# angela000/DQNFlappyBird

Hardware: AMD Instinct MI355X
Metric: env steps/sec (whole node) + DQN grad-steps/sec, 80x80x4 batch=32 (higher is better)
Workload: dtype f32

## Files before the change

### dqnflappybird_amd/csrc/fb_qnet.hip

```cpp
#include <math.h>
#include <stdlib.h>
#include "fb_common.h"

#ifndef FK_ABL
#define FK_ABL 0
#endif
#ifndef BW_ABL
#define BW_ABL 0
#endif

namespace {

typedef float f32x16 __attribute__((ext_vector_type(16)));

constexpr int OFF_W1 = 0, OFF_B1 = 8192, OFF_W2 = 8224, OFF_B2 = 40992, OFF_W3 = 41056, OFF_B3 = 77920,
              OFF_WF1 = 77984;
constexpr int CONV_PARAMS = OFF_WF1;
#include "fb_head.h"
#include "fb_sampler.h"
#include "fb_gather.h"
constexpr int MAXTB = 256;


struct Slice { const float *params; const uint8_t *states; int s_off, count; const uint16_t *w1s; int fshift; };
// ... 1607 lines not shown

__global__ __launch_bounds__(256) void noisy_sigma_init_kernel(float *__restrict__ p, NoisyNet N) {
    const int q = OFF_WF1 + blockIdx.x * 256 + threadIdx.x;
    if (q >= N.n) return;
    p[N.n + q - OFF_WF1] = noisy_layer(N, q).sig;
}

__device__ __forceinline__ float env_noise_f(uint32_t seed_lo, uint32_t seed_hi, uint32_t c0, uint32_t step_lo, uint32_t step_hi) {
    const fb_u4 r = fb_philox(seed_lo, seed_hi, c0, step_lo, FB_STREAM_ENV_NOISE, step_hi);
    const float u1 = ((r.x >> 8) + 1) * (1.0f / 16777216.0f), u2 = (r.y >> 8) * (1.0f / 16777216.0f);
    const float z = sqrtf(-2.f * logf(u1)) * cosf(6.28318530717958647692f * u2);
    return copysignf(sqrtf(fabsf(z)), z);
}

__global__ __launch_bounds__(256) void env_noise_sigsplit_kernel(const float *__restrict__ sig, uint4 *__restrict__ wsp, int FC, const AdamDev *ad,
                                                                const int *seen) {
    if (*seen == ad->applies) return;
    const int id = blockIdx.x * 256 + threadIdx.x;
    if (id < 200 * FC) wsplit_item(sig, wsp, FC, IT_CONV + id);
}

struct EnvScale { const uint16_t *a3; const float *h3; size_t pl; uint16_t *out; int n, nz; uint32_t seed_lo, seed_hi, step_lo, step_hi;
                  const AdamDev *ad; int *seen; unsigned *ovf; };
__global__ __launch_bounds__(256) void env_noise_scale_kernel(EnvScale a) {
    if (blockIdx.x == 0 && threadIdx.x == 0) *a.seen = a.ad->applies;
    const int id = blockIdx.x * 256 + threadIdx.x, e = min(id / 800, a.n - 1), k = 2 * (id - (id / 800) * 800);
    const bool on = id < a.n * 800;
    const size_t o = (size_t)e * 1600 + k;
    float x0, x1;
    if (a.a3) {
        const uint32_t hi = *reinterpret_cast<const uint32_t *>(a.a3 + o), lo = *reinterpret_cast<const uint32_t *>(a.a3 + a.pl + o);
        const f32x2 h = __builtin_convertvector(__builtin_bit_cast(f16x2, hi), f32x2), l = __builtin_convertvector(__builtin_bit_cast(f16x2, lo), f32x2);
        x0 = fmaf(l.x, F16_LO_UNSCALE, h.x); x1 = fmaf(l.y, F16_LO_UNSCALE, h.y);
    } else { x0 = a.h3[o]; x1 = a.h3[o + 1]; }
    const uint32_t c = (uint32_t)e * (uint32_t)a.nz + (uint32_t)k;
    const float y0 = x0 * env_noise_f(a.seed_lo, a.seed_hi, c, a.step_lo, a.step_hi), y1 = x1 * env_noise_f(a.seed_lo, a.seed_hi, c + 1u, a.step_lo, a.step_hi);
    uint32_t hi, lo;
    split2x2(y0, y1, hi, lo);
    if (on) { *reinterpret_cast<uint32_t *>(a.out + o) = hi; *reinterpret_cast<uint32_t *>(a.out + a.pl + o) = lo; }
    note_overflow(on && out_of_f16_range(y0, y1, 0.f, 0.f), a.ovf);
}

struct EnvNoiseHead {
    const float *hf, *ht; int stot, nks;
    const float *P; NetOff hoff; const float *sig; NetOff off; NoisyNet N;
    int n, FC, A; C51Sup sup; float *q; uint8_t *actions; float epsilon; uint32_t seed_lo, seed_hi, step_lo, step_hi;
    const int32_t *key_of; uint32_t stream;
};
constexpr int ENH_WAVES = 8;
template <int AT> struct EnhLds { static constexpr int KC = AT == 2 ? 64 : 16, PER = (KC * AT * 64 + 511) / 512, PERV = (KC * 64 + 511) / 512; };
template <int AT, bool DUEL>
__global__ __launch_bounds__(64 * ENH_WAVES) void env_noise_head_kernel(EnvNoiseHead H) {
    constexpr int KC = EnhLds<AT>::KC, PER = EnhLds<AT>::PER, PERV = EnhLds<AT>::PERV, WQ = KC * AT * 64;
    __shared__ float lw[2 * WQ + (DUEL ? KC * 64 : 0)];
    const int tid = threadIdx.x, lane = tid & 63, row = blockIdx.x * ENH_WAVES + (tid >> 6);
    const bool live = row < H.n;
    const int smp = live ? row : H.n - 1;
    const int A = AT == MAXA ? H.A : AT, N = H.sup.N, AN = A * N, il = lane < N ? lane : N - 1, FC = H.FC;
    const bool on = lane < N;
    const int key = H.key_of ? H.key_of[smp] : smp;
    const uint32_t base = (uint32_t)key * (uint32_t)H.N.nz;
    auto draw = [&](int k) { return env_noise_f(H.seed_lo, H.seed_hi, base + (uint32_t)k, H.step_lo, H.step_hi); };
    const NoisyLayer L0 = H.N.l[0], LV = H.N.l[1], LQ = H.N.l[DUEL ? 2 : 1];
    float lg[AT], ns[AT], nv = 0.f;
#pragma unroll
    for (int a = 0; a < AT; a++) { lg[a] = 0.f; ns[a] = 0.f; }
    float x = 0.f, xq = 0.f, xv = 0.f;
    for (int k0 = 0; k0 < FC; k0 += KC) {
        const int cq = KC * AN, cv = KC * N;
        const float *__restrict__ gm = H.P + H.hoff.wq + (size_t)k0 * AN, *__restrict__ gq = H.sig + H.off.wq + (size_t)k0 * AN;
        const float *__restrict__ gv = H.sig + H.off.wv + (size_t)k0 * N;
        float tm[PER], tq[PER], tv[DUEL ? PERV : 1];
#pragma unroll
        for (int r = 0; r < PER; r++) { const int i = min(tid + r * 512, cq - 1); tm[r] = gm[i]; tq[r] = gq[i]; }
        if (DUEL) {
#pragma unroll
            for (int r = 0; r < PERV; r++) tv[r] = gv[min(tid + r * 512, cv - 1)];
        }
        if (k0 % 64 == 0) {
            const int j = k0 + lane;
            float v = H.hf[(size_t)smp * FC + j], t[FC1_KS];
#pragma unroll
            for (int ks = 1; ks < FC1_KS; ks++) {
                const float y = H.hf[((size_t)(ks < H.nks ? ks : 0) * H.stot + smp) * FC + j];
                t[ks] = ks < H.nks ? y : 0.f;
            }
#pragma unroll
            for (int ks = 1; ks < FC1_KS; ks++) v += t[ks];
            const float pre = v + H.P[H.hoff.bf1 + j];
            float tt = H.ht[(size_t)smp * FC + j];
#pragma unroll
            for (int ks = 1; ks < FC1_SP_KS; ks++) tt += H.ht[((size_t)ks * H.stot + smp) * FC + j];
            x = fmaxf(pre + draw(L0.eout + j) * (tt + H.sig[H.off.bf1 + j]), 0.f);
            xq = x * draw(LQ.ein + j);
            xv = DUEL ? x * draw(LV.ein + j) : 0.f;
        }
        __syncthreads();
#pragma unroll
        for (int r = 0; r < PER; r++) { const int i = tid + r * 512; if (i < cq) { lw[i] = tm[r]; lw[WQ + i] = tq[r]; } }
        if (DUEL) {
#pragma unroll
            for (int r = 0; r < PERV; r++) { const int i = tid + r * 512; if (i < cv) lw[2 * WQ + i] = tv[r]; }
        }
        __syncthreads();
        const int kl = k0 % 64;
#pragma unroll 8
        for (int k = 0; k < KC; k++) {
            const float xs = rdlane(x, kl + k), xqs = rdlane(xq, kl + k);
#pragma unroll
            for (int a = 0; a < AT; a++) {
                const int o = k * AN + (a < A ? a : 0) * N + il;
                lg[a] = fmaf(xs, lw[o], lg[a]);
                ns[a] = fmaf(xqs, lw[WQ + o], ns[a]);
            }
            if (DUEL) nv = fmaf(rdlane(xv, kl + k), lw[2 * WQ + k * N + il], nv);
        }
    }
#pragma unroll
    for (int a = 0; a < AT; a++) lg[a] += H.P[H.hoff.bq + (a < A ? a : 0) * N + il];
    float nq[AT], mean = 0.f;
#pragma unroll
    for (int a = 0; a < AT; a++) {
        const int o = (a < A ? a : 0) * N + il;
        nq[a] = draw(LQ.eout + o) * (ns[a] + H.sig[H.off.bq + o]);
        if (a < A) mean += nq[a];
    }
    if (DUEL) {
        mean /= (float)A;
        const float vn = draw(LV.eout + il) * (nv + H.sig[H.off.bv + il]);
#pragma unroll
        for (int a = 0; a < AT; a++) lg[a] += (vn + nq[a]) - mean;
    } else {
#pragma unroll
        for (int a = 0; a < AT; a++) lg[a] += nq[a];
    }
    float qv[AT];
    const float z = H.sup.vmin + (float)(on ? lane : 0) * H.sup.dz;
    c51_q<AT>(lg, on, z, qv);
    if (lane == 0 && live) {
#pragma unroll
        for (int a = 0; a < AT; a++) if (a < A) H.q[(size_t)smp * A + a] = qv[a];
        int best = 0;
#pragma unroll
        for (int a = 1; a < AT; a++) if (a < A && qv[a] > qv[best]) best = a;
        const fb_u4 o = fb_philox(H.seed_lo, H.seed_hi, (uint32_t)key, H.step_lo, H.stream, H.step_hi);
        const float u = (float)(o.x >> 8) * (1.0f / 16777216.0f);
        if (u <= H.epsilon) best = (int)(((unsigned long long)o.y * (unsigned)A) >> 32);
        H.actions[smp] = (uint8_t)best;
    }
}

typedef float f32x4 __attribute__((ext_vector_type(4)));
struct FkArgs { Slices sl; const float *h3; float *hf; float *qpart; int FC, A, dueling, stot; NetOff off; };
constexpr int FK_ROW = 204;

__global__ __launch_bounds__(512) void fc1_fk_kernel(FkArgs a) {
    __shared__ float ast[8 * 16 * FK_ROW];
    __shared__ float red[8 * 4 * 64];
    const Slice s = a.sl.s[blockIdx.z];
    const int M = s.count, m0 = blockIdx.x * 16, n0 = blockIdx.y * 16;
    if (m0 >= M) return;
    const int lane = threadIdx.x & 63, wave = threadIdx.x >> 6, r = lane & 15, g = lane >> 4;
    const int kw = wave * 200;
    const float *bcol = s.params + OFF_WF1 + (size_t)(kw + 50 * g) * a.FC + n0 + r;
    float bv[50];
#pragma unroll
    for (int t = 0; t < 50; t++) bv[t] = bcol[(size_t)(FK_ABL == 2 ? 0 : t) * a.FC];
    float hb = s.params[a.off.bf1 + n0 + r], hw[MAXA + 1];
#pragma unroll
    for (int c = 0; c < MAXA; c++) hw[c] = s.params[a.off.wq + (n0 + r) * a.A + (c < a.A ? c : 0)];
    hw[MAXA] = s.params[(a.dueling ? a.off.wv : a.off.bf1) + n0 + r];
    float *mine = ast + wave * 16 * FK_ROW;
    float4 st[13];
#pragma unroll
    for (int i = 0; i < 13; i++) {
        const int idx = lane + 64 * i, row = idx < 800 ? idx / 50 : 0, c4 = idx < 800 ? idx - row * 50 : 0;
        const int mr = m0 + row < M ? m0 + row : M - 1;
        st[i] = *reinterpret_cast<const float4 *>(a.h3 + (size_t)(s.s_off + mr) * 1600 + kw + 4 * (FK_ABL == 3 ? 0 : c4));
    }
#pragma unroll
    for (int i = 0; i < 13; i++) {
        const int idx = lane + 64 * i, row = idx / 50, c4 = idx - row * 50;
        if (idx < 800) *reinterpret_cast<float4 *>(mine + row * FK_ROW + 4 * c4) = st[i];
    }
    __builtin_amdgcn_wave_barrier();
    asm volatile("s_waitcnt lgkmcnt(0)" ::: "memory");
    const float *arow = mine + r * FK_ROW + 50 * g;
    f32x4 acc0 = {0.f, 0.f, 0.f, 0.f}, acc1 = {0.f, 0.f, 0.f, 0.f};
    float2 av[25];
#pragma unroll
    for (int t = 0; t < 25; t++) av[t] = *reinterpret_cast<const float2 *>(arow + 2 * t);
#pragma unroll
    for (int t = 0; t < 25; t++) { keep(av[t].x); keep(av[t].y); }
#pragma unroll
    for (int t = 0; t < (FK_ABL == 1 ? 1 : 25); t++) {
        acc0 = __builtin_amdgcn_mfma_f32_16x16x4f32(rbf(av[t].x, a.sl.rb), rbf(bv[2 * t], a.sl.rb), acc0, 0, 0, 0);
        acc1 = __builtin_amdgcn_mfma_f32_16x16x4f32(rbf(av[t].y, a.sl.rb), rbf(bv[2 * t + 1], a.sl.rb), acc1, 0, 0, 0);
    }
#pragma unroll
    for (int q = 0; q < 4; q++) red[(wave * 4 + q) * 64 + lane] = acc0[q] + acc1[q];
    __syncthreads();
    if (threadIdx.x >= 256) return;
    const int reg = threadIdx.x >> 6, row = 4 * g + reg, col = r, mr = m0 + row, unit = n0 + col;
    float v = red[reg * 64 + lane];
#pragma unroll
    for (int w = 1; w < 8; w++) v += red[(w * 4 + reg) * 64 + lane];
    const bool live = mr < M;
    const size_t srow = (size_t)s.s_off + (live ? mr : M - 1);
    if (live) a.hf[srow * a.FC + unit] = v;
    if (!a.qpart || FK_ABL == 4) return;
    const float h = fmaxf(v + hb, 0.f);
    const int qs = a.A + 1;
    float *qo = a.qpart + (srow * (size_t)gridDim.y + blockIdx.y) * qs;
#pragma unroll
    for (int c = 0; c <= MAXA; c++) {
        if (c < a.A || (c == a.A && a.dueling)) {
            float x = h * (c == a.A ? hw[MAXA] : hw[c]);
#pragma unroll
            for (int o = 8; o > 0; o >>= 1) x += __shfl_xor(x, o, 16);
            if (col == 0 && live) qo[c] = x;
        }
    }
}

struct Bw1Args {
    int algo, B, FC, A, dueling, stot, n_dx, rb;
    NetOff off;
    const float *params, *pnext, *ptarget;
    const float *hf, *qpart, *h3;
    const uint8_t *act; const float *rew; const uint8_t *term; const float *isw;
    double gamma;
    float *grad, *dh3, *loss, *abs_err, *y_out;
    AdamDev *adam; int tick;
    FbGate gate;
};
constexpr int BW_DX_ROW = 4;
constexpr int BW_DW_ROW = 36;

template <int AT, bool DX>
__device__ __forceinline__ void fc1_bwd2_body(const Bw1Args &L, float *smem) {
    const int tid = threadIdx.x, lane = tid & 63, wave = tid >> 6, B = L.B, FC = L.FC, A = AT == MAXA ? L.A : AT;
    const float *P = L.params;
    float (*dadv)[MAXA] = reinterpret_cast<float (*)[MAXA]>(smem);
    float *dv = smem + MAXTB * MAXA, *lterm = dv + MAXTB, *dadv2 = lterm + MAXTB, *big = dadv2 + 2 * MAXTB;
    const bool lead = blockIdx.x == 0;
    const bool dbl = L.algo == FB_ALGO_DOUBLE;
    const int qs = A + 1, ntile = FC >> 4;
    constexpr bool dx_role = DX;
    const int mt = dx_role ? blockIdx.x / 50 : 0, t2 = dx_role ? 0 : blockIdx.x - L.n_dx, nt = t2 / 7, kg = t2 - nt * 7;
    const int kt = dx_role ? blockIdx.x - mt * 50 : kg * 8 + wave;
    auto unit_params = [&](int n, float &bias, float (&wq)[AT], float &wv) {
        bias = P[L.off.bf1 + n];
        wv = P[(L.dueling ? L.off.wv : L.off.bf1) + n];
#pragma unroll
        for (int c = 0; c < AT; c++) wq[c] = P[L.off.wq + n * A + (c < A ? c : 0)];
    };
    float pre_hf[32], pre_bias, pre_wq[AT], pre_wv, pre_a[16];
    float4 pre_w[8];
    if constexpr (DX) {
        const int ch = FC < 512 ? FC : 512, n = tid < ch ? tid : 0;
#pragma unroll
        for (int q = 0; q < 32; q++) { const int bq_ = mt * 32 + q; pre_hf[q] = L.hf[(size_t)(bq_ < B ? bq_ : 0) * FC + n]; }
        unit_params(n, pre_bias, pre_wq, pre_wv);
        const int kh = ch / 16, nbeg = wave * (ch / 8) + (lane >> 5) * kh;
        const float *brun = P + OFF_WF1 + (size_t)(kt * 32 + (lane & 31)) * FC + nbeg;
#pragma unroll
        for (int q = 0; q < 8; q++) pre_w[q] = *reinterpret_cast<const float4 *>(brun + (4 * q < kh ? 4 * q : 0));
#pragma unroll
        for (int q = 0; q < 16; q++) pre_a[q] = 0.f;
#pragma unroll
        for (int q = 0; q < 2; q++) { const int mr = mt * 32 + drow(2 * (wave & 7) + q, lane); pre_a[q] = L.h3[(size_t)(mr < B ? mr : 0) * 1600 + kt * 32 + (lane & 31)]; }
    } else {
        const int c = tid & 31;
#pragma unroll
        for (int q = 0; q < 2; q++) { const int b = (tid >> 5) + 16 * q; pre_hf[q] = L.hf[(size_t)(b < B ? b : 0) * FC + nt * 32 + c]; }
#pragma unroll
        for (int q = 2; q < 32; q++) pre_hf[q] = 0.f;
        unit_params(nt * 32 + c, pre_bias, pre_wq, pre_wv);
        const int ktc = kt < 50 ? kt : 0;
#pragma unroll
        for (int t = 0; t < 16; t++) { const int b = 2 * t + (lane >> 5); pre_a[t] = L.h3[(size_t)(b < B ? b : 0) * 1600 + ktc * 32 + (lane & 31)]; }
#pragma unroll
        for (int q = 0; q < 8; q++) pre_w[q] = make_float4(0.f, 0.f, 0.f, 0.f);
    }
    float bqs[AT], bqn[AT], bq3[AT];
#pragma unroll
    for (int c = 0; c < AT; c++) { const int cc = c < A ? c : 0; bqs[c] = L.params[L.off.bq + cc]; bqn[c] = L.pnext[L.off.bq + cc]; bq3[c] = L.ptarget[L.off.bq + cc]; }
    const int bvo = L.dueling ? L.off.bv : L.off.bq;
    float bvs = L.params[bvo], bvn = L.pnext[bvo], bv3 = L.ptarget[bvo];
    for (int b0 = 0; b0 < (BW_ABL == 1 ? 0 : B); b0 += 32) {
        const int b = b0 + (tid >> 4), j = tid & 15, bc = b < B ? b : 0;
        float rf = L.rew[bc], isw = L.isw ? L.isw[bc] : 1.f;
        int termb = L.term[bc], a_b = L.act[bc];
        float x0[2][AT + 1], x1[2][AT + 1], x2[2][AT + 1];
#pragma unroll
        for (int u = 0; u < 2; u++) {
            const int tile = j + 16 * u, tc = tile < ntile ? tile : 0;
            const float *q0 = L.qpart + ((size_t)bc * ntile + tc) * qs;
            const size_t rs = (size_t)ntile * qs;
#pragma unroll
            for (int c = 0; c <= AT; c++) {
                const int cc = c < qs ? c : 0;
                x0[u][c] = q0[cc]; x1[u][c] = q0[(size_t)B * rs + cc]; x2[u][c] = q0[(size_t)(dbl ? 2 * B : 0) * rs + cc];
            }
        }
        keep(rf); keep(isw); keep(termb); keep(a_b);
        float qsv[AT + 1], qnv[AT + 1], q3v[AT + 1];
#pragma unroll
        for (int c = 0; c <= AT; c++) {
            keep(x0[0][c]); keep(x1[0][c]); keep(x2[0][c]); keep(x0[1][c]); keep(x1[1][c]); keep(x2[1][c]);
            const bool on = c < A || (c == A && L.dueling), on0 = on && j < ntile, on1 = on && j + 16 < ntile;
            qsv[c] = (on0 ? x0[0][c] : 0.f) + (on1 ? x0[1][c] : 0.f);
            qnv[c] = (on0 ? x1[0][c] : 0.f) + (on1 ? x1[1][c] : 0.f);
            q3v[c] = (on0 ? x2[0][c] : 0.f) + (on1 ? x2[1][c] : 0.f);
        }
        for (int tile = j + 32; tile < ntile; tile += 16) {
            const float *q0 = L.qpart + ((size_t)bc * ntile + tile) * qs;
            const size_t rs = (size_t)ntile * qs;
#pragma unroll
            for (int c = 0; c <= AT; c++) {
                const int cc = c < qs ? c : 0;
                const bool on = c < A || (c == A && L.dueling);
                const float y0 = q0[cc], y1 = q0[(size_t)B * rs + cc], y2 = q0[(size_t)(dbl ? 2 * B : 0) * rs + cc];
                qsv[c] += on ? y0 : 0.f; qnv[c] += on ? y1 : 0.f; q3v[c] += on ? y2 : 0.f;
            }
        }
#pragma unroll
        for (int c = 0; c <= AT; c++)
#pragma unroll
            for (int o = 8; o > 0; o >>= 1) { qsv[c] += __shfl_xor(qsv[c], o, 16); qnv[c] += __shfl_xor(qnv[c], o, 16); q3v[c] += __shfl_xor(q3v[c], o, 16); }
        float vs = 0.f, vn = 0.f, v3 = 0.f;
#pragma unroll
        for (int c = 0; c <= AT; c++) { vs = c == A ? qsv[c] : vs; vn = c == A ? qnv[c] : vn; v3 = c == A ? q3v[c] : v3; }
        auto fin = [&](float (&qv)[AT + 1], float vshare, const float (&bq)[AT], float bvv) {
            float mean = 0.f;
#pragma unroll
            for (int c = 0; c < AT; c++) { qv[c] = c < A ? qv[c] + bq[c] : 0.f; mean += c < A ? qv[c] : 0.f; }
            const float V = vshare + bvv;
            mean /= (float)A;
#pragma unroll
            for (int c = 0; c < AT; c++) qv[c] = L.dueling ? V + (qv[c] - mean) : qv[c];
        };
        fin(qsv, vs, bqs, bvs);
        fin(qnv, vn, bqn, bvn);
        fin(q3v, v3, bq3, bv3);
        float sel;
        {
            int am = 0;
#pragma unroll
            for (int c = 1; c < AT; c++) if (c < A && qnv[c] > qnv[am]) am = c;
            float seld = q3v[0], selm = qnv[0];
#pragma unroll
            for (int c = 1; c < AT; c++) { seld = c == am ? q3v[c] : seld; selm = c < A ? fmaxf(selm, qnv[c]) : selm; }
            sel = dbl ? seld : selm;
        }
        if (L.algo != FB_ALGO_PER) isw = 1.f;
        const double rr = rf == 0.1f ? 0.1 : (double)rf;
        const double yd = termb ? rr : rr + L.gamma * (double)sel;
        const float y = (float)yd;
// ... 1553 lines not shown
    return FB_OK;
}

static void resplit_now(fb_qnet *h, int which, hipStream_t st) {
    const int items = wsplit_items(h->FC);
    hipLaunchKernelGGL(wsplit_kernel, dim3((items + 255) / 256), dim3(256), 0, st, h->params[which], h->wsp[which], h->FC,
                       (const unsigned *)&h->adam->pver[which], (const unsigned *)&h->adam->wver[which]);
    hipLaunchKernelGGL(mark_split_kernel, dim3(1), dim3(1), 0, st, h->adam, which);
}

extern "C" int fb_qnet_init_params(fb_qnet_t h, int which, uint64_t seed, void *stream) {
    FB_REQUIRE(h && (which == 0 || which == 1), "fb_qnet_init_params: bad argument");
    hipLaunchKernelGGL(init_params_kernel, dim3((unsigned)((h->n + 255) / 256)), dim3(256), 0, fb_stream(stream),
                       master(h, which), h->n, h->off, h->FC, h->sup.N ? h->A * h->sup.N : h->A, h->arch == FB_ARCH_DUELING || is_c51d(h), (uint32_t)seed,
                       (uint32_t)(seed >> 32));
    if (is_c51d(h)) {
        const float b = 0.01f;
        uint32_t bits;
        memcpy(&bits, &b, 4);
        FB_CHECK_HIP(hipMemsetD32Async((hipDeviceptr_t)(master(h, which) + h->off.bv), (int)bits, (size_t)h->sup.N, fb_stream(stream)));
    }
    if (h->noisy)
        hipLaunchKernelGGL(noisy_sigma_init_kernel, dim3((unsigned)((h->n - OFF_WF1 + 255) / 256)), dim3(256), 0, fb_stream(stream), h->mst[which], h->nnet);
    noisy_materialise(h, which, 0, false, fb_stream(stream));
    env_noise_invalidate(h, which, fb_stream(stream));
    c51d_fold(h, which, fb_stream(stream));
    hipLaunchKernelGGL(w1_split_kernel, dim3(32), dim3(256), 0, fb_stream(stream), h->params[which], h->w1s[which], &h->adam->pver[which]);
    resplit_now(h, which, fb_stream(stream));
    FB_LAUNCH_CHECK();
    return FB_OK;
}

extern "C" int fb_qnet_load_params(fb_qnet_t h, int which, const float *flat, void *stream) {
    FB_REQUIRE(h && flat && (which == 0 || which == 1), "fb_qnet_load_params: bad argument");
    FB_CHECK_HIP(hipMemcpyAsync(master(h, which), flat, sizeof(float) * (size_t)h->ntot, hipMemcpyDeviceToDevice, fb_stream(stream)));
    noisy_materialise(h, which, 0, false, fb_stream(stream));
    env_noise_invalidate(h, which, fb_stream(stream));
    hipLaunchKernelGGL(w1_split_kernel, dim3(32), dim3(256), 0, fb_stream(stream), h->params[which], h->w1s[which], &h->adam->pver[which]);
    c51d_fold(h, which, fb_stream(stream));
    resplit_now(h, which, fb_stream(stream));
    FB_LAUNCH_CHECK();
    return FB_OK;
}

extern "C" int fb_qnet_store_params(fb_qnet_t h, int which, float *flat, void *stream) {
    FB_REQUIRE(h && flat && (which == 0 || which == 1), "fb_qnet_store_params: bad argument");
    FB_CHECK_HIP(hipMemcpyAsync(flat, master(h, which), sizeof(float) * (size_t)h->ntot, hipMemcpyDeviceToDevice, fb_stream(stream)));
    return FB_OK;
}

extern "C" int fb_qnet_get_adam_state(fb_qnet_t h, float *m, float *v, float *beta_pows_host) {
    FB_REQUIRE(h, "fb_qnet_get_adam_state: NULL handle");
    FB_CHECK_HIP(hipDeviceSynchronize());
    const size_t nb = sizeof(float) * (size_t)h->ntot;
    if (m) FB_CHECK_HIP(hipMemcpy(m, h->adam_m, nb, hipMemcpyDeviceToDevice));
    if (v) FB_CHECK_HIP(hipMemcpy(v, h->adam_v, nb, hipMemcpyDeviceToDevice));
    if (beta_pows_host) {
        AdamDev a;
        FB_CHECK_HIP(hipMemcpy(&a, h->adam, sizeof(a), hipMemcpyDeviceToHost));
        beta_pows_host[0] = a.b1pow; beta_pows_host[1] = a.b2pow;
    }
    return FB_OK;
}

extern "C" int fb_qnet_set_adam_state(fb_qnet_t h, const float *m, const float *v, const float *beta_pows_host) {
    FB_REQUIRE(h, "fb_qnet_set_adam_state: NULL handle");
    FB_CHECK_HIP(hipDeviceSynchronize());
    const size_t nb = sizeof(float) * (size_t)h->ntot;
    if (m) FB_CHECK_HIP(hipMemcpy(h->adam_m, m, nb, hipMemcpyDeviceToDevice));
    if (v) FB_CHECK_HIP(hipMemcpy(h->adam_v, v, nb, hipMemcpyDeviceToDevice));
    if (beta_pows_host) {
        AdamDev a;
        FB_CHECK_HIP(hipMemcpy(&a, h->adam, sizeof(a), hipMemcpyDeviceToHost));
        a.b1pow = beta_pows_host[0]; a.b2pow = beta_pows_host[1];
        FB_CHECK_HIP(hipMemcpy(h->adam, &a, sizeof(a), hipMemcpyHostToDevice));
    }
    return FB_OK;
}

enum KernelId {
    K_CONV1 = 0, K_CONV2, K_CONV3, K_FC1, K_HEAD, K_LOSS, K_FC1_BWD, K_CONV3_BWD, K_CONV2_BWD, K_CONV1_DW, K_SLAB, K_ADAM,
    K_COUNT
};

struct Plan {
    Slices sl; int ns;
    bool nib;
    uint8_t *actions; float epsilon; uint64_t seed, step;
    bool train;
    int algo, B; const uint8_t *s, *a, *t; const float *r, *isw; double gamma;
    float *loss, *abs_err, *y, *G; bool apply_adam, tick;
    FbHeadRider *head_rider;
    const FbSampleRider *sample_rider;
    const FbRingSrc *ring;
    const FbSplitCtx *split;
    bool any_rows;
    float *probs;
    bool no_head;
};

#include <type_traits>
template <int V> using IntTag = std::integral_constant<int, V>;
template <class F> static void with_nsp(int nsp, F f) { if (nsp == 3) f(IntTag<3>{}); else f(IntTag<1>{}); }
template <class F> static void with_bool(bool b, F f) { if (b) f(std::true_type{}); else f(std::false_type{}); }
template <class F> static void with_actions(int A, F f) { if (A == 2) f(IntTag<2>{}); else f(IntTag<MAXA>{}); }

template <class T> static void put_seed_words(T &c, uint64_t seed, uint64_t step) {
    c.seed_lo = (uint32_t)seed; c.seed_hi = (uint32_t)(seed >> 32);
    c.step_lo = (uint32_t)step; c.step_hi = (uint32_t)(step >> 32);
}

struct PlanCtx {
    int only; hipStream_t st;
    int maxc, total;
    bool big, trunk, fused, c51;
    int nsp, stot; size_t pl1, pl2;
};
static bool runs(const PlanCtx &c, int id) { return c.only < 0 || c.only == id; }

static PlanCtx plan_ctx(const fb_qnet *h, const Plan &p, int only, hipStream_t st) {
    PlanCtx c{only, st, 0, 0};
    for (int z = 0; z < p.ns; z++) { if (p.sl.s[z].count > c.maxc) c.maxc = p.sl.s[z].count; c.total += p.sl.s[z].count; }
    c.big = c.maxc >= 256 || p.any_rows;
    c.nsp = p.train ? h->nsplit_train : h->nsplit;
    c.stot = 3 * h->max_batch; c.pl1 = (size_t)c.stot * 3200; c.pl2 = (size_t)c.stot * 1600;
    c.trunk = p.ring != nullptr;
    c.fused = c.big && p.nib && !p.train && !c.trunk && p.ns == 1;
    c.c51 = h->sup.N > 0;
    return c;
}

static C23T trunk_args(fb_qnet *h, const Plan &p, const PlanCtx &c, SplitJob *job) {
    C23T c23t;
    memset(job, 0, sizeof(*job)); memset(&c23t, 0, sizeof(c23t));
    job->FC = h->FC;
    c23t.sl = p.sl; c23t.p1 = h->p1; c23t.h2 = h->h2; c23t.h3 = h->h3; c23t.ovf = &h->adam->ovf;
    for (int z = 0; z < p.ns; z++) {
        const int which = p.sl.s[z].params == h->params[1] ? 1 : 0;
        c23t.w[z] = h->wsp[which] + WSP_W2;
        if (c.only < 0) {
            job->params[which] = h->params[which]; job->wsp[which] = h->wsp[which];
            job->pver[which] = &h->adam->pver[which]; job->wverc[which] = &h->adam->wverc[which];
            c23t.pver[which] = &h->adam->pver[which]; c23t.wverc[which] = &h->adam->wverc[which];
        }
    }
    return c23t;
}

static void ring_trunk(fb_qnet *h, const Plan &p, const PlanCtx &c) {
    SplitJob job;
    C23T c23t = trunk_args(h, p, c, &job);
    if (c.big) { c23t.a3s = h->a3s; c23t.pl3 = c.pl2; }
    c23t.ring = *p.ring; c23t.p1o = h->p1; c23t.amax = h->amax; c23t.ring_fo = h->ring_fo;
    const bool w16 = c.maxc * p.ns <= 256;
    const bool nst = p.ring->c.nstep > 1;
    with_nsp(c.nsp, [&](auto ns) { with_bool(w16, [&](auto w) { with_bool(nst, [&](auto nv) {
        constexpr bool W16 = decltype(w)::value;
        hipLaunchKernelGGL((conv23_t_kernel<decltype(ns)::value, true, W16, decltype(nv)::value>), dim3(c.maxc, p.ns), dim3(W16 ? 1024 : 512), 0, c.st, c23t);
    }); }); });
}

static int large_pass(fb_qnet *h, const Plan &p, const PlanCtx &c, int *z) {
    const int z0 = *z;
    int z1 = z0 + 1;
    while (z1 < p.ns && p.sl.s[z1].params == p.sl.s[z0].params && p.sl.s[z1].count == p.sl.s[z0].count && p.sl.s[z1].s_off == p.sl.s[z1 - 1].s_off + p.sl.s[z1 - 1].count) z1++;
    const Slice s0 = p.sl.s[z0];
    const int which = s0.params == h->params[1] ? 1 : 0, row0 = s0.s_off, rows = s0.count * (z1 - z0);
    const unsigned *pver = c.only < 0 ? &h->adam->pver[which] : nullptr;
    unsigned *wver = c.only < 0 ? &h->adam->wver[which] : nullptr;
    Slice sl = s0;
    sl.count = rows;
    C1Side side;
    memset(&side, 0, sizeof(side));
    if (z1 - z0 > 1) { side.per = s0.count; side.st1 = p.sl.s[z0 + 1].states; side.st2 = z1 - z0 > 2 ? p.sl.s[z0 + 2].states : p.sl.s[z0 + 1].states; }
    if (p.train) { side.p1 = h->p1; side.amax = h->amax; }
    const int t1p = (rows * 100 + 7) / 8, gsp = min(256, (t1p + C1_WAVES - 1) / C1_WAVES);
    if (!c.trunk && !c.fused && runs(c, K_CONV1))
        hipLaunchKernelGGL(conv1_sp_kernel, dim3(gsp), dim3(64 * C1_WAVES), 0, c.st, sl, (const uint8_t *)h->zeros, h->a1s, c.pl1, c.nsp, h->wsp[which], h->FC, pver, (const unsigned *)wver, side, &h->adam->ovf);
    C23Args c23{h->a1s + (size_t)row0 * 3200, c.pl1, h->wsp[which] + WSP_W2, s0.params + OFF_B2, s0.params + OFF_B3, h->a3s + (size_t)row0 * 1600, c.pl2, rows, pver, wver, c.only < 0 ? &h->adam->wverc[which] : nullptr,
                p.train ? h->h2 + (size_t)row0 * 1600 : nullptr, p.train ? h->h3 + (size_t)row0 * 1600 : nullptr,
                s0.states, s0.w1s, s0.params + OFF_B1, s0.params, h->wsp[which], h->FC, &h->adam->ovf};
    Fc1Args af{h->a3s + (size_t)row0 * 1600, c.pl2, h->zeros, h->wsp[which] + WSP_WF1, (c.fused ? h->hf_act : h->hf) + (size_t)row0 * h->FC, c.stot, rows, h->FC,
               c.fused ? pver : nullptr, c.fused ? wver : nullptr, nullptr, 0,
               c.fused ? head_base(h, s0.params) + h->off.bf1 : nullptr, c.fused ? h->hp_act : nullptr, c.fused ? (int)(h->hoff.n - h->off.bf1) : 0,
               c.fused && p.split && c.only < 0 ? &p.split->f->trunk_done : nullptr, p.split ? p.split->seq : 0};
    if (c.trunk && z1 < p.ns && rows % 128 == 0) {
        int z2 = z1 + 1;
        while (z2 < p.ns && p.sl.s[z2].params == p.sl.s[z1].params && p.sl.s[z2].s_off == p.sl.s[z2 - 1].s_off + p.sl.s[z2 - 1].count) z2++;
        const Slice sn = p.sl.s[z1];
        if (z2 == p.ns && sn.s_off == row0 + rows && sn.params != s0.params) {
            int rows2 = 0;
            for (int z = z1; z < z2; z++) rows2 += p.sl.s[z].count;
            af.w2 = h->wsp[sn.params == h->params[1] ? 1 : 0] + WSP_WF1; af.m_split = rows; af.M = rows + rows2;
            z1 = z2;
        }
    }
    *z = z1;
    const dim3 gc((rows + 4) / 5), gf(((af.M + 127) / 128) * (h->FC / 64) * FC1_SP_KS);
    if (c.fused && p.split && c.only < 0 && gc.x > 256 && gc.x % 256 != 0) { c23.round_flag = &p.split->f->last_round; c23.round_val = p.split->seq; c23.round_blk = (int)(gc.x / 256) * 256; }
    with_nsp(c.nsp, [&](auto ns) {
        if (!c.trunk && runs(c, K_CONV2))
            with_bool(c.fused, [&](auto fu) { hipLaunchKernelGGL((conv23_sp_kernel<decltype(ns)::value, 5, decltype(fu)::value>), gc, dim3(512), 0, c.st, c23); });
        if (runs(c, K_FC1)) hipLaunchKernelGGL(fc1_sp_kernel<decltype(ns)::value>, gf, dim3(256), 0, c.st, af);
    });
    if (c.fused && (c.only < 0 || c.only == K_FC1) && (long long)af.hp_n > (long long)gf.x * 256) {
        const size_t done = (size_t)gf.x * 256;
        FB_CHECK_HIP(hipMemcpyAsync(h->hp_act + done, af.hp_src + done, sizeof(float) * ((size_t)af.hp_n - done), hipMemcpyDeviceToDevice, c.st));
    }
    return FB_OK;
}

static void small_forward(fb_qnet *h, const Plan &p, const PlanCtx &c) {
    if (!c.trunk) {
        SplitJob job;
        const C23T c23t = trunk_args(h, p, c, &job);
        const int t1 = (c.maxc * 100 + 7) / 8;
        if (runs(c, K_CONV1))
            with_bool(p.nib, [&](auto nib) { hipLaunchKernelGGL(conv1_pool_kernel<decltype(nib)::value>, dim3((t1 + 3) / 4, 1, p.ns), dim3(256), 0, c.st, p.sl, h->p1, h->amax, job); });
        if (runs(c, K_CONV2))
            with_nsp(c.nsp, [&](auto ns) { hipLaunchKernelGGL((conv23_t_kernel<decltype(ns)::value, false>), dim3(c.maxc, p.ns), dim3(512), 0, c.st, c23t); });
    }
    if (runs(c, K_FC1)) {
        FkArgs fa;
        fa.sl = p.sl; fa.h3 = h->h3; fa.hf = h->hf; fa.qpart = p.train && !c.c51 ? h->qpart : nullptr; fa.FC = h->FC; fa.A = h->A;
        fa.dueling = h->arch == FB_ARCH_DUELING; fa.stot = c.stot; fa.off = h->off;
        hipLaunchKernelGGL(fc1_fk_kernel, dim3((c.maxc + 15) / 16, h->FC / 16, p.ns), dim3(512), 0, c.st, fa);
    }
}

static void launch_dist_head(const fb_qnet *h, const C51HeadArgs &H, int rows, hipStream_t st) {
    with_actions(h->A, [&](auto a) {
        if (is_qr(h)) hipLaunchKernelGGL(qr_head_kernel<decltype(a)::value>, dim3((rows + 3) / 4), dim3(256), 0, st, H);
        else hipLaunchKernelGGL(c51_head_kernel<decltype(a)::value>, dim3((rows + 3) / 4), dim3(256), 0, st, H);
    });
}

static void head_stage(fb_qnet *h, const Plan &p, const PlanCtx &c) {
    if (c.c51 && !p.train && !p.no_head && runs(c, K_HEAD)) {
        C51HeadArgs H;
        H.sl = p.sl; H.nslices = p.ns; H.params = nullptr;
        for (int z = 0; z < p.ns; z++) H.sl.s[z].params = head_base(h, p.sl.s[z].params);
        C51Core &C = H.c;
        C.hf = c.fused ? h->hf_act : h->hf; C.stot = c.stot; C.nks = c.big ? FC1_SP_KS : 1; C.q = h->q; C.probs = p.probs; C.FC = h->FC; C.A = h->A;
        C.off = h->hoff; C.sup = h->sup; C.actions = p.actions; C.epsilon = p.epsilon;
        put_seed_words(C, p.seed, p.step); C.key_of = nullptr; C.stream = FB_STREAM_EPS;
        if (p.head_rider) {
            memset(p.head_rider, 0, sizeof(*p.head_rider));
            p.head_rider->c.hf = C.hf; p.head_rider->c.stot = c.stot; p.head_rider->c.nks = C.nks;
            p.head_rider->params = c.fused ? h->hp_act - h->off.bf1 : H.sl.s[0].params;
        } else launch_dist_head(h, H, c.total, c.st);
    }
    if (!c.c51 && !(!c.big && p.train) && runs(c, K_HEAD)) {
        HeadArgs H;
        H.sl = p.sl; H.nslices = p.ns;
        HeadCore &C = H.c;
        C.hf = c.fused ? h->hf_act : h->hf; C.stot = c.stot; C.nks = c.big ? FC1_SP_KS : 1; C.q = h->q; C.FC = h->FC; C.A = h->A;
        C.dueling = h->arch == FB_ARCH_DUELING; C.off = h->off; C.actions = p.actions; C.epsilon = p.epsilon;
        put_seed_words(C, p.seed, p.step);
        if (p.head_rider) { p.head_rider->c = C; p.head_rider->params = c.fused ? h->hp_act - h->off.bf1 : p.sl.s[0].params; p.head_rider->on = 1; p.head_rider->on_arrival = nullptr; p.head_rider->arrival_val = 0; }
        else hipLaunchKernelGGL(head_kernel, dim3((c.total + 3) / 4), dim3(256), 0, c.st, H);
    }
}

static void loss_stage(fb_qnet *h, const Plan &p, const PlanCtx &c) {
    const int B = p.B, FC = h->FC;
    if (!c.c51) {
        LossArgs L;
        L.algo = p.algo; L.B = B; L.FC = FC; L.A = h->A; L.dueling = h->arch == FB_ARCH_DUELING; L.off = h->off;
        L.params = h->params[0]; L.q = h->q; L.hf = h->hf; L.stot = c.stot; L.nks = FC1_SP_KS; L.act = p.a; L.rew = p.r; L.term = p.t; L.isw = p.isw;
        L.gamma = p.gamma; L.grad = p.G; L.dhf = h->dhf; L.loss = p.loss; L.abs_err = p.abs_err; L.y_out = p.y; L.gmax = h->gmax;
        L.adam = h->adam; L.tick = p.tick;
        hipLaunchKernelGGL(loss_head_kernel, dim3(FC / 16), dim3(256), 0, c.st, L);
        return;
    }
    const bool pw = is_per_algo(p.algo);
    auto shared = [&](auto &L) {
        L.B = B; L.FC = FC; L.A = h->A; L.nks = c.big ? FC1_SP_KS : 1; L.stot = c.stot; L.off = h->hoff;
        L.p_on = head_base(h, h->params[0]); L.p_next = head_base(h, p.sl.s[1].params);
        L.p_tgt = head_base(h, p.ns > 2 ? p.sl.s[2].params : p.sl.s[1].params);
        L.hf = h->hf; L.act = p.a; L.rew = p.r; L.term = p.t; L.gamma = p.gamma;
        L.dl = h->c51_dl; L.xs = h->c51_xs; L.lterm = h->c51_lt; L.dhf = h->dhf;
        L.isw = pw ? p.isw : nullptr; L.abs_err = pw ? p.abs_err : nullptr;
    };
    with_actions(h->A, [&](auto a) { with_bool(pw, [&](auto w) {
        if (is_qr(h)) {
            QRLossArgs L;
            shared(L);
            L.algo = is_double_qr(p.algo) ? FB_ALGO_QR_DOUBLE : FB_ALGO_QR; L.N = h->sup.N; L.kappa = h->kappa;
            hipLaunchKernelGGL((qr_loss_kernel<decltype(a)::value, decltype(w)::value>), dim3((B + 3) / 4), dim3(256), 0, c.st, L);
        } else {
            C51LossArgs L;
            shared(L);
            L.algo = is_double_c51(p.algo) ? FB_ALGO_C51_DOUBLE : FB_ALGO_C51; L.sup = h->sup;
            hipLaunchKernelGGL((c51_loss_kernel<decltype(a)::value, decltype(w)::value>), dim3((B + 3) / 4), dim3(256), 0, c.st, L);
        }
    }); });
    const C51GradArgs gA{B, FC, h->A, h->sup.N, h->off, h->c51_dl, h->c51_xs, h->c51_lt, h->dhf, p.a, p.G, p.loss, h->gmax, h->adam, p.tick};
    if (is_c51d(h)) hipLaunchKernelGGL(c51d_grad_kernel, dim3(FC / 16), dim3(256), 0, c.st, gA);
    else hipLaunchKernelGGL(c51_grad_kernel, dim3(FC / 16), dim3(256), 0, c.st, gA);
}

static void fc1_backward(fb_qnet *h, const Plan &p, const PlanCtx &c) {
    const int B = p.B, FC = h->FC;
    if (!c.big && !c.c51) {
        const int ndx1 = ((B + 31) / 32) * 50;
        Bw1Args L;
        L.algo = p.algo; L.B = B; L.FC = FC; L.A = h->A; L.dueling = h->arch == FB_ARCH_DUELING; L.stot = c.stot; L.n_dx = ndx1; L.off = h->off;
// ... 495 lines not shown
```

Measured before the change: 11.13 million.

## Halve fc1 LDS staging and overlap second-half loads with MFMAs

Restructures the fc1 fused kernel into two K-halves. The LDS staging buffer shrinks to half width with an XOR swizzle, and the reduction scratch reuses that buffer. Weight and activation loads for the second half are issued between the first half's MFMAs, with a waves_per_eu hint to lift occupancy. A separate change turns off the 1024-thread trunk variant for small split plans. The aim is to hide global-load latency and cut LDS and register use, at the cost of more complex scheduling and possible register pressure.

After: 10.24 million. 0.92x the previous value.

```diff
diff --git a/dqnflappybird_amd/csrc/fb_qnet.hip b/dqnflappybird_amd/csrc/fb_qnet.hip
--- a/dqnflappybird_amd/csrc/fb_qnet.hip
+++ b/dqnflappybird_amd/csrc/fb_qnet.hip
@@ -1783,59 +1783,88 @@
 
 typedef float f32x4 __attribute__((ext_vector_type(4)));
 struct FkArgs { Slices sl; const float *h3; float *hf; float *qpart; int FC, A, dueling, stot; NetOff off; };
-constexpr int FK_ROW = 204;
-
-__global__ __launch_bounds__(512) void fc1_fk_kernel(FkArgs a) {
+constexpr int FK_ROW = 104;
+
+__global__ __launch_bounds__(512) __attribute__((amdgpu_waves_per_eu(6))) void fc1_fk_kernel(FkArgs a) {
     __shared__ float ast[8 * 16 * FK_ROW];
-    __shared__ float red[8 * 4 * 64];
     const Slice s = a.sl.s[blockIdx.z];
     const int M = s.count, m0 = blockIdx.x * 16, n0 = blockIdx.y * 16;
     if (m0 >= M) return;
     const int lane = threadIdx.x & 63, wave = threadIdx.x >> 6, r = lane & 15, g = lane >> 4;
     const int kw = wave * 200;
-    const float *bcol = s.params + OFF_WF1 + (size_t)(kw + 50 * g) * a.FC + n0 + r;
-    float bv[50];
-#pragma unroll
-    for (int t = 0; t < 50; t++) bv[t] = bcol[(size_t)(FK_ABL == 2 ? 0 : t) * a.FC];
+    const float *wrow = s.params + OFF_WF1 + n0;
+    const unsigned bcol = 4u * (unsigned)((kw + 50 * g) * a.FC + r);
+    auto wld = [&](int t) { return *reinterpret_cast<const float *>(reinterpret_cast<const char *>(wrow + (size_t)(FK_ABL == 2 ? 0 : t) * a.FC) + bcol); };
+    float b0[26], b1[24];
+#pragma unroll
+    for (int t = 0; t < 26; t++) b0[t] = wld(t);
+    const float *h3s = a.h3 + (size_t)(s.s_off + m0) * 1600;
+    const int mlast = M - 1 - m0;
+    const int sl0 = lane < 52 ? lane : 51, sl1 = lane < 48 ? lane : 47;
+    auto src = [&](int row, int slot, int t0) {
+        const int gg = (slot & 3) ^ ((row >> 3) << 1);
+        const unsigned o = 4u * (unsigned)(kw + 50 * gg + 2 * (FK_ABL == 3 ? 0 : t0 + (slot >> 2)));
+        return reinterpret_cast<const float2 *>(reinterpret_cast<const char *>(h3s + (size_t)(row < mlast ? row : mlast) * 1600) + o);
+    };
+    float *mine = ast + wave * 16 * FK_ROW;
+    float2 s0[16], s1[16];
+#pragma unroll
+    for (int i = 0; i < 16; i++) s0[i] = *src(i, sl0, 0);
+#pragma unroll
+    for (int i = 0; i < 16; i++) *reinterpret_cast<float2 *>(mine + i * FK_ROW + 2 * sl0) = s0[i];
+    __builtin_amdgcn_wave_barrier();
+    asm volatile("s_waitcnt lgkmcnt(0)" ::: "memory");
+    const float *arow = mine + r * FK_ROW + 2 * (g ^ ((r >> 3) << 1));
+    f32x4 acc0 = {0.f, 0.f, 0.f, 0.f}, acc1 = {0.f, 0.f, 0.f, 0.f};
+    float2 a0[13], a1[12];
+#pragma unroll
+    for (int t = 0; t < 13; t++) a0[t] = *reinterpret_cast<const float2 *>(arow + 8 * t);
+#pragma unroll
+    for (int t = 0; t < 13; t++) { keep(a0[t].x); keep(a0[t].y); }
+#pragma unroll
+    for (int t = 0; t < (FK_ABL == 1 ? 1 : 13); t++) {
+        acc0 = __builtin_amdgcn_mfma_f32_16x16x4f32(rbf(a0[t].x, a.sl.rb), rbf(b0[2 * t], a.sl.rb), acc0, 0, 0, 0);
+        acc1 = __builtin_amdgcn_mfma_f32_16x16x4f32(rbf(a0[t].y, a.sl.rb), rbf(b0[2 * t + 1], a.sl.rb), acc1, 0, 0, 0);
+        if (t >= 2) {
+            const int k = t - 2;
+            b1[2 * k] = wld(26 + 2 * k);
+            b1[2 * k + 1] = wld(27 + 2 * k);
+            if (k == 10) { b1[22] = wld(48); b1[23] = wld(49); }
+            s1[k] = *src(k, sl1, 13);
+            if (k < 5) s1[11 + k] = *src(11 + k, sl1, 13);
+        }
+        __builtin_amdgcn_sched_barrier(0);
+    }
+    __builtin_amdgcn_wave_barrier();
+    asm volatile("" ::: "memory");
+#pragma unroll
+    for (int i = 0; i < 16; i++) *reinterpret_cast<float2 *>(mine + i * FK_ROW + 2 * sl1) = s1[i];
+    __builtin_amdgcn_wave_barrier();
+    asm volatile("s_waitcnt lgkmcnt(0)" ::: "memory");
     float hb = s.params[a.off.bf1 + n0 + r], hw[MAXA + 1];
 #pragma unroll
     for (int c = 0; c < MAXA; c++) hw[c] = s.params[a.off.wq + (n0 + r) * a.A + (c < a.A ? c : 0)];
     hw[MAXA] = s.params[(a.dueling ? a.off.wv : a.off.bf1) + n0 + r];
-    float *mine = ast + wave * 16 * FK_ROW;
-    float4 st[13];
-#pragma unroll
-    for (int i = 0; i < 13; i++) {
-        const int idx = lane + 64 * i, row = idx < 800 ? idx / 50 : 0, c4 = idx < 800 ? idx - row * 50 : 0;
-        const int mr = m0 + row < M ? m0 + row : M - 1;
-        st[i] = *reinterpret_cast<const float4 *>(a.h3 + (size_t)(s.s_off + mr) * 1600 + kw + 4 * (FK_ABL == 3 ? 0 : c4));
-    }
-#pragma unroll
-    for (int i = 0; i < 13; i++) {
-        const int idx = lane + 64 * i, row = idx / 50, c4 = idx - row * 50;
-        if (idx < 800) *reinterpret_cast<float4 *>(mine + row * FK_ROW + 4 * c4) = st[i];
+#pragma unroll
+    for (int t = 0; t < 12; t++) a1[t] = *reinterpret_cast<const float2 *>(arow + 8 * t);
+#pragma unroll
+    for (int t = 0; t < 12; t++) { keep(a1[t].x); keep(a1[t].y); }
+#pragma unroll
+    for (int t = 0; t < (FK_ABL == 1 ? 0 : 12); t++) {
+        acc0 = __builtin_amdgcn_mfma_f32_16x16x4f32(rbf(a1[t].x, a.sl.rb), rbf(b1[2 * t], a.sl.rb), acc0, 0, 0, 0);
+        acc1 = __builtin_amdgcn_mfma_f32_16x16x4f32(rbf(a1[t].y, a.sl.rb), rbf(b1[2 * t + 1], a.sl.rb), acc1, 0, 0, 0);
     }
     __builtin_amdgcn_wave_barrier();
-    asm volatile("s_waitcnt lgkmcnt(0)" ::: "memory");
-    const float *arow = mine + r * FK_ROW + 50 * g;
-    f32x4 acc0 = {0.f, 0.f, 0.f, 0.f}, acc1 = {0.f, 0.f, 0.f, 0.f};
-    float2 av[25];
-#pragma unroll
-    for (int t = 0; t < 25; t++) av[t] = *reinterpret_cast<const float2 *>(arow + 2 * t);
-#pragma unroll
-    for (int t = 0; t < 25; t++) { keep(av[t].x); keep(av[t].y); }
-#pragma unroll
-    for (int t = 0; t < (FK_ABL == 1 ? 1 : 25); t++) {
-        acc0 = __builtin_amdgcn_mfma_f32_16x16x4f32(rbf(av[t].x, a.sl.rb), rbf(bv[2 * t], a.sl.rb), acc0, 0, 0, 0);
-        acc1 = __builtin_amdgcn_mfma_f32_16x16x4f32(rbf(av[t].y, a.sl.rb), rbf(bv[2 * t + 1], a.sl.rb), acc1, 0, 0, 0);
-    }
-#pragma unroll
-    for (int q = 0; q < 4; q++) red[(wave * 4 + q) * 64 + lane] = acc0[q] + acc1[q];
+    asm volatile("" ::: "memory");
+    float *red = ast;
+#pragma unroll
+    for (int q = 0; q < 4; q++) mine[q * 64 + lane] = acc0[q] + acc1[q];
     __syncthreads();
     if (threadIdx.x >= 256) return;
     const int reg = threadIdx.x >> 6, row = 4 * g + reg, col = r, mr = m0 + row, unit = n0 + col;
     float v = red[reg * 64 + lane];
 #pragma unroll
-    for (int w = 1; w < 8; w++) v += red[(w * 4 + reg) * 64 + lane];
+    for (int w = 1; w < 8; w++) v += red[w * 16 * FK_ROW + reg * 64 + lane];
     const bool live = mr < M;
     const size_t srow = (size_t)s.s_off + (live ? mr : M - 1);
     if (live) a.hf[srow * a.FC + unit] = v;
@@ -3695,7 +3724,7 @@
     C23T c23t = trunk_args(h, p, c, &job);
     if (c.big) { c23t.a3s = h->a3s; c23t.pl3 = c.pl2; }
     c23t.ring = *p.ring; c23t.p1o = h->p1; c23t.amax = h->amax; c23t.ring_fo = h->ring_fo;
-    const bool w16 = c.maxc * p.ns <= 256;
+    const bool w16 = c.maxc * p.ns <= 256 && !(p.split && c.only < 0 && c.maxc < 128);
     const bool nst = p.ring->c.nstep > 1;
     with_nsp(c.nsp, [&](auto ns) { with_bool(w16, [&](auto w) { with_bool(nst, [&](auto nv) {
         constexpr bool W16 = decltype(w)::value;
```
